# Simple-Robotics/LoIK

Hardware: AMD Instinct MI355X
Metric: IK solves/sec to 1e-6 residual, Talos humanoid, batch=65536 per GPU (higher is better)
Workload: dtype f64

## Files before the change

loik_amd/csrc/loik_flat.hpp:

```cpp
#pragma once

#include "loik_lean.hpp"

namespace loikb {

constexpr int FLAT_RED = 8;
constexpr int FLAT_PART = 8;
constexpr int FLAT_JMP = 5;
constexpr int FLAT_MAXA = 16;
constexpr int FOLDW = 10;
constexpr int FLAT_COUNTERS_SLOT_HITS = 12;
constexpr int FLAT_NA_SMALL = 10;
constexpr int FSLOT_ROWS = 8;

struct FlatLane {
  int depth;
  int size;
  int jmp[FLAT_JMP];
  int anc[FLAT_MAXA];
  int red[FLAT_RED];
  int helper;
  int part[FLAT_PART];
};

enum : int { FC_LANE = 0, FC_B = 1, FC_Y = 7, FC_ATY = 13, FC_ATYW = 19, FC_ATBW = 25, FC_DY = 31, FC_DLT = 37, FC_ATYF = 43, FC_AW = 49, FC_A = 85,
              FC_VC = FC_DLT , FCD = 121 };
enum : int { FI_BNORM = 0, FI_TGIN, FI_STY, FI_TOLP, FI_TOLD, FI_DYQP, FI_ATDY, FI_UBP, FI_LBM, FI_C1, FI_C2, FI_PRIMAL, FI_DUAL, FI_DX,
             FI_DZ, FI_MULAST, FI_RED , FISC = FI_RED + 16 };

template <int NA>
__host__ __device__ constexpr int flat_xregion()
{
  int n = XROWS * 9;
  if (NA * WAVE + 2 > n) n = NA * WAVE + 2;
  if (WAVE * FOLDW > n) n = WAVE * FOLDW;
  return (n + 1) & ~1;
}
template <int NA> __host__ __device__ constexpr int flat_off_wl() { return flat_xregion<NA>(); }
template <int NA> __host__ __device__ constexpr int flat_off_nbuf() { return flat_off_wl<NA>() + 2 * (NA + 1) * WAVE; }
template <int NA> __host__ __device__ constexpr int flat_off_pbuf() { return flat_off_nbuf<NA>() + WAVE + 2; }
template <int NA> __host__ __device__ constexpr int flat_off_rbuf() { return flat_off_pbuf<NA>() + WAVE + 2; }
template <int NA> __host__ __device__ constexpr int flat_off_tail() { return flat_off_rbuf<NA>() + WAVE; }

template <typename T, int NA>
__host__ __device__ __forceinline__ size_t flat_lds_bytes(int nc, int G, bool a_shared, bool has_hv)
{
  (void)a_shared;
  const size_t per_inst = (size_t)nc * FCD + FISC;
  const size_t n = (size_t)flat_off_tail<NA>() + (has_hv ? (size_t)WAVE * 6 : 0) + (size_t)(WAVE / G) * per_inst;
  return (n * sizeof(T) + 15) & ~(size_t)15;
}

__device__ __forceinline__ size_t fslotA_at(int idx, int ndec, int dsl, int fblk, int G, int k, int jlane)
{
  (void)G;
  return ((size_t)idx * ndec + dsl) * fblk + (size_t)jlane * 8 + k;
}
__device__ __forceinline__ size_t fslotW_at(int idx, int ndec, int dsl, int fblk, int col)
{
  return ((size_t)idx * ndec + dsl) * fblk + col;
}

template <typename T>
__device__ __forceinline__ void se3_compose_left(const T* Ra, const T* ta, T* R, T* t)
{
  T Rn[9], tn[3];
#pragma unroll
  for (int i = 0; i < 3; ++i) {
#pragma unroll
    for (int j = 0; j < 3; ++j) Rn[3 * i + j] = Ra[3 * i] * R[j] + Ra[3 * i + 1] * R[3 + j] + Ra[3 * i + 2] * R[6 + j];
    tn[i] = ta[i] + Ra[3 * i] * t[0] + Ra[3 * i + 1] * t[1] + Ra[3 * i + 2] * t[2];
  }
#pragma unroll
  for (int k = 0; k < 9; ++k) R[k] = Rn[k];
#pragma unroll
  for (int k = 0; k < 3; ++k) t[k] = tn[k];
}

template <typename T>
__device__ __forceinline__ void flat_world_placement(T* xb, int lane, int jlane, const unsigned int* jrow4, int njmp, T* R, T* t)
{
#pragma unroll 1
  for (int r = 0; r < njmp; ++r) {
    {
      const int jr = (int)(((r < 4 ? jrow4[0] : jrow4[1]) >> (8 * (r & 3))) & 0xFFu);
      T Ra[9], ta[3];
      tail_sync();
      if (jlane < 9) xb[WAVE * 9 + jlane] = (jlane == 0 || jlane == 4 || jlane == 8) ? T(1) : T(0);
#pragma unroll
      for (int k = 0; k < 9; ++k) xb[lane * 9 + k] = R[k];
      tail_sync();
#pragma unroll
      for (int k = 0; k < 9; ++k) Ra[k] = xb[jr * 9 + k];
      tail_sync();
      if (jlane < 3) xb[WAVE * 9 + jlane] = T(0);
#pragma unroll
      for (int k = 0; k < 3; ++k) xb[lane * 9 + k] = t[k];
      tail_sync();
#pragma unroll
      for (int k = 0; k < 3; ++k) ta[k] = xb[jr * 9 + k];
      se3_compose_left(Ra, ta, R, t);
    }
  }
  tail_sync();
}

template <typename T>
__device__ __forceinline__ void flat_subtree_sum(T* rows, int lane, int jlane, int lim, int size, int nscan, const T* x, T* S)
{
  tail_sync();
  if (jlane < 6) rows[WAVE * 6 + jlane] = T(0);
  T B[6];
#pragma unroll
  for (int k = 0; k < 6; ++k) { B[k] = x[k]; S[k] = T(0); }
  int pos = lane;
  for (int k = 0; k < nscan; ++k) {
    tail_sync();
#pragma unroll
    for (int c = 0; c < 6; ++c) rows[lane * 6 + c] = B[c];
    tail_sync();
    const bool take = (size >> k) & 1;
    const int ra = take ? pos : WAVE;
    const int nx = lane + (1 << k);
    const int rb = nx < lim ? nx : WAVE;
    T a[6], b[6];
#pragma unroll
    for (int c = 0; c < 6; ++c) a[c] = rows[ra * 6 + c];
#pragma unroll
    for (int c = 0; c < 6; ++c) b[c] = rows[rb * 6 + c];
#pragma unroll
    for (int c = 0; c < 6; ++c) { S[c] += a[c]; B[c] += b[c]; }
    pos += take ? (1 << k) : 0;
  }
}

template <typename T>
__device__ __forceinline__ void flat_path_sum(T* rows, int lane, int jlane, const unsigned int* jrow4, int njmp, T* y)
{
  tail_sync();
  if (jlane < 6) rows[WAVE * 6 + jlane] = T(0);
#pragma unroll 1
  for (int r = 0; r < njmp; ++r) {
    {
      const int jr = (int)(((r < 4 ? jrow4[0] : jrow4[1]) >> (8 * (r & 3))) & 0xFFu);
      tail_sync();
#pragma unroll
      for (int c = 0; c < 6; ++c) rows[lane * 6 + c] = y[c];
      tail_sync();
      T a[6];
#pragma unroll
      for (int c = 0; c < 6; ++c) a[c] = rows[jr * 6 + c];
#pragma unroll
      for (int c = 0; c < 6; ++c) y[c] += a[c];
    }
  }
}

template <typename T>
__device__ __forceinline__ void actinv_force(const T* R, const T* t, const T* F, T* o)
{
  T c[3], d[3];
  cross3(t, F, c);
#pragma unroll
  for (int k = 0; k < 3; ++k) d[k] = F[3 + k] - c[k];
  mat3t_vec(R, F, o);
  mat3t_vec(R, d, o + 3);
}

template <typename T, int NMAX>
__device__ __forceinline__ void flat_fold8(T* rows, int lane, int gbase, int jlane, int lgG, const T* in, T* out)
{
  tail_sync();
  T* row = rows + lane * FOLDW;
#pragma unroll
  for (int q = 0; q < 8; ++q) row[q] = in[q];
  tail_sync();
  const int q = jlane & 7;
  const bool ismax = q < NMAX;
  const int nparts = 1 << (lgG - 3);
  {
    const T* col = rows + (gbase + (jlane >> 3)) * FOLDW + q;
    T a[8];
#pragma unroll
    for (int u = 0; u < 8; ++u) a[u] = col[u * nparts * FOLDW];
    const T m = tmax(tmax(tmax(a[0], a[1]), tmax(a[2], a[3])), tmax(tmax(a[4], a[5]), tmax(a[6], a[7])));
    T sm = a[0];
#pragma unroll
    for (int u = 1; u < 8; ++u) sm += a[u];
    row[8] = (NMAX >= 8 || ismax) ? m : sm;
  }
  tail_sync();
  {
    const T* col = rows + (gbase + q) * FOLDW + 8;
    T a[8];
#pragma unroll
    for (int p = 0; p < 8; ++p) a[p] = (p < 4 || lgG > 5) ? col[p * 8 * FOLDW] : T(0);
    const T m = tmax(tmax(tmax(a[0], a[1]), tmax(a[2], a[3])), tmax(tmax(a[4], a[5]), tmax(a[6], a[7])));
    T sm = a[0];
#pragma unroll
    for (int p = 1; p < 8; ++p) sm += a[p];
    row[9] = (NMAX >= 8 || ismax) ? m : sm;
  }
  tail_sync();
#pragma unroll
  for (int u = 0; u < 8; ++u) out[u] = rows[(gbase + u) * FOLDW + 9];
}

__device__ __forceinline__ unsigned int opaque(unsigned int x) { asm volatile("" : "+v"(x)); return x; }
__device__ __forceinline__ int unpack8(const unsigned int* w, int k) { return (int)((opaque(w[k >> 2]) >> (8 * (k & 3))) & 0xFFu); }
__device__ __forceinline__ int unpack16(const unsigned int* w, int k) { return (int)((opaque(w[k >> 1]) >> (16 * (k & 1))) & 0xFFFFu); }
// ... 537 lines not shown
        put_rows();
        tail_sync();
        scan_step(kk);
      }
      if (kk >= nscan) {
        tail_sync();
        part_v();
      } else {
        put_rows();
        tail_sync();
        const int wv = 1 << kk;
        const bool take0 = (size >> kk) & 1, take1 = (size >> (kk + 1)) & 1;
        const int p1 = pos + (take0 ? wv : 0);
        const int r0 = take0 ? pos : WAVE, r1 = take1 ? p1 : WAVE, r2 = take1 ? p1 + wv : WAVE;
        T a[6], b[6], c2[6];
#pragma unroll
        for (int c = 0; c < 6; ++c) a[c] = xb[r0 * 6 + c];
#pragma unroll
        for (int c = 0; c < 6; ++c) b[c] = xb[r1 * 6 + c];
#pragma unroll
        for (int c = 0; c < 6; ++c) c2[c] = xb[r2 * 6 + c];
        part_v();
#pragma unroll
        for (int c = 0; c < 6; ++c) SEn[c] += a[c] + (b[c] + c2[c]);
      }
      tail_sync();
      TAIL_TP(4)
#pragma unroll
      for (int k = 0; k < 6; ++k) Fw[k] = (P.rho + href_s) * SEn[k] - P.rho * SE[k];
      if (has_hv) {
#pragma unroll
        for (int k = 0; k < 6; ++k) Fw[k] -= shv[lane * 6 + k];
      }
      for (int c = 0; c < L.nc; ++c) {
        const T* c_ = cdi + c * cs;
        const T m = cmask(c);
#pragma unroll
        for (int k = 0; k < 6; ++k) Fw[k] += m * c_[FC_ATYF + k];
      }
      actinv_force(R0, t0, Fw, fi);
      si = dot6_halves(Sw, Fw);
#pragma unroll
      for (int k = 0; k < 6; ++k) SE[k] = SEn[k];
    }
    TAIL_TP(5)
    {
      T df[6];
#pragma unroll
      for (int k = 0; k < 6; ++k) df[k] = fi[k] - f[k];
      l_dfis = mass * inf6(df);
      si += w;
      l_stf = tabs(si);
      l_dstf = tabs(si - s);
      s = si;
#pragma unroll
      for (int k = 0; k < 6; ++k) f[k] = fi[k];
    }
    TAIL_TP(3)
    T red[8];
    {
      T in[8] = {tmax(l_prt, l_prs), tmax(l_dualv, l_stf), tmax(l_dvis, l_dnu), l_dz,
                 tmax(l_dfis, tmax(l_dyis, l_dw)), tmax(l_dg, l_dstf), l_up, l_lm};
      flat_fold8<T, 6>(xb, lane, gbase, jlane, lgG, in, red);
    }
    T ntol_p = T(0), ntol_d = T(0);
    if (P.tol_rel != T(0)) {
      T in2[8] = {tmax(l_av, l_nu), tmax(tmax(l_hrefv, l_g), l_stf), T(0), T(0), T(0), T(0), T(0), T(0)}, r2[8];
      flat_fold8<T, 8>(xb, lane, gbase, jlane, lgG, in2, r2);
      ntol_p = r2[0]; ntol_d = r2[1];
    }
    TAIL_TP(6)
    const T primal = red[0], dual = red[1], dx = red[2], dz = red[3], dyqp = red[4], atdy = red[5], ubp = red[6], lbm = red[7];
    const T mu_used = mu;
    const bool fixed = P.mode & MODE_FIXED_ITERS;
    const bool in_tail = (status & ST_TAIL) != 0;
    const bool logic = act && !fixed && !in_tail;
    const T tol_p = P.tol_abs + P.tol_rel * tmax(ntol_p, isc[FI_BNORM]);
    const T tol_d = P.tol_abs + P.tol_rel * tmax(ntol_d, P.Hv_inf_norm);
    const int itn = iter + (act ? 1 : 0);
    const bool conv = logic && (primal < tol_p) && (dual < tol_d);
    const bool feas_chk = logic && itn > 1;
    const bool c1 = atdy <= P.tol_primal_inf * dyqp, c2 = (ubp + lbm) <= P.tol_primal_inf * dyqp;
    const bool infeas = feas_chk && c1 && c2;
    const bool enter_tail = infeas && !conv;
    const bool upd = logic && !conv && !infeas;
    const bool mu_up = upd && (primal > T(10) * dual), mu_dn = upd && !mu_up && (dual > T(10) * primal);
    const bool tail_stop = !(dx >= P.tol_tail_solve || dz >= P.tol_tail_solve) || itn >= P.max_iter;
    const bool stop = act && (conv || ((enter_tail || in_tail) && tail_stop) || ((upd || fixed) && itn + 1 >= P.max_iter));
    iter = itn;
    status |= (conv ? ST_CONVERGED : 0) | (infeas ? ST_PRIMAL_INF : 0) | (enter_tail ? ST_TAIL : 0) | (stop ? ST_DONE : 0);
    tail_it = enter_tail ? 0 : (act && in_tail ? tail_it + 1 : tail_it);
    mu = mu_up ? mu * T(10) : (mu_dn ? mu * T(0.1) : mu);
    kexp += (mu_up ? 1 : 0) - (mu_dn ? 1 : 0);
    nflip += (mu_up || mu_dn) ? 1 : 0;
    done = done || stop;
    const bool finishing = stop;
    const bool leaving = done && has_inst;
    if (LOG) {
      T inl[8] = {l_prt, l_prs, l_stf, l_dualv, T(0), T(0), T(0), T(0)}, rl[8];
      flat_fold8<T, 8>(xb, lane, gbase, jlane, lgG, inl, rl);
      const int row = itn - 1;
      if (act && !in_tail && jlane == 0 && row < Bf.log_cap) {
        const double vals[9] = {(double)rl[0], (double)rl[1], (double)primal, (double)rl[2], (double)rl[3], (double)dual,
                                (double)mu_used, (double)(P.mu_scale * mu_used), (double)mu_used};
#pragma unroll
        for (int l = 0; l < 9; ++l) Bf.log[((size_t)l * Bf.log_B + lidx) * Bf.log_cap + row] = vals[l];
      }
    }
    if (__any(finishing || enter_tail)) {
      if ((finishing || enter_tail) && jlane == 0) {
        isc[FI_PRIMAL] = primal; isc[FI_DUAL] = dual; isc[FI_DX] = dx; isc[FI_DZ] = dz; isc[FI_MULAST] = mu_used;
        if (logic) { isc[FI_TOLP] = tol_p; isc[FI_TOLD] = tol_d; }
        if (feas_chk) {
          isc[FI_C1] = (T)(c1 ? 1 : 0); isc[FI_C2] = (T)(c2 ? 1 : 0); isc[FI_DYQP] = dyqp; isc[FI_ATDY] = atdy; isc[FI_UBP] = ubp; isc[FI_LBM] = lbm;
        }
      }
    }
    if (__any(finishing)) {
      T in1[8] = {l_prt, l_prs, l_stf, l_dvis, l_dnu, l_dfis, l_dyis, l_dw}, in2[8] = {l_av, l_nu, l_hrefv, l_g, l_dualv, T(0), T(0), T(0)};
      T r1[8], r2[8];
      flat_fold8<T, 8>(xb, lane, gbase, jlane, lgG, in1, r1);
      flat_fold8<T, 8>(xb, lane, gbase, jlane, lgG, in2, r2);
      if (finishing && jlane == 0) {
#pragma unroll
        for (int k = 0; k < 8; ++k) isc[FI_RED + k] = r1[k];
#pragma unroll
        for (int k = 0; k < 5; ++k) isc[FI_RED + 8 + k] = r2[k];
      }
      tail_sync();
    }
    if (leaving) {
      store_instance();
      need_load = true;
    }
    TAIL_TP(7)
  }
#ifdef LOIKB_TAIL_PROF
  if (blockIdx.x == 0 && threadIdx.x == 0) {
    for (int k = 0; k < 8; ++k) g_tail_prof[k] = prof_[k];
    for (int k = 8; k < 12; ++k) g_tail_prof[2 + k] = prof_[k];
    g_tail_prof[8] = n_wave_iters;
    g_tail_prof[9] = (clock64() - clk0_) * 100000ull / (wall_clock64() - wall0_ + 1);
  }
#endif
  if (lane == 0) atomicAdd(&Bf.counters[5], n_wave_iters);
  if (jlane == 0) {
    atomicAdd(&Bf.counters[6], n_slot_loads >> 16);
    atomicAdd(&Bf.counters[FLAT_COUNTERS_SLOT_HITS], n_slot_hits);
    atomicOr(&Bf.counters[LEAN_DECADES_SEEN], n_slot_loads & 0xFFFFu);
  }
}

template <typename T, int NA>
__global__ void __launch_bounds__(WAVE)
k_fslots(const Params<T> P, const Bufs<T> Bf, const JointDesc* __restrict__ jd, const TailTopo* __restrict__ topo,
         const int* __restrict__ child_list, const FlatLane* __restrict__ fl, int maxdepth, int nanc, int frows, int njmp,
         const int* __restrict__ slots, int nslots, int G, T* __restrict__ fslots, int kexp_lo, int ndec, int dw0, int nw,
         unsigned int* __restrict__ fmask)
{
  extern __shared__ __attribute__((aligned(16))) unsigned char smem_raw[];
  const Layout& L = P.L;
  constexpr int HX = 22;
  T* xch = reinterpret_cast<T*>(smem_raw);
  T* swt = xch + (WAVE + 1) * HX;
  T* ata_l = swt + (WAVE + 1) * 6;
  T* mutab = ata_l + (size_t)(WAVE / G) * P.L.nc * 21;
  T* lb = xch;
  const int lane = threadIdx.x;
  const int ipw = WAVE / G;
  const int sub = lane / G, jlane = lane % G, gbase = sub * G;
  const int nblk = gridDim.x, xcd = blockIdx.x & 7, rnd = blockIdx.x >> 3;
  const int blk = xcd * (nblk >> 3) + (xcd < (nblk & 7) ? xcd : (nblk & 7)) + rnd;
  const int idx = blk * ipw + sub;
  const bool has_inst = idx < nslots;
  const bool isj_lane = jlane < L.nb;
  const bool isj = has_inst && isj_lane;
  const int jl = isj_lane ? jlane : 0;
  const int sidx = slots[has_inst ? idx : 0];
  char* ip = lane_ptr<T>(Bf.tiles, L, sidx);
  int depth, fcol, arow[NA];
  T Sw[6];
  bool has_parent;
  int cslot;
  T base0[21];
  {
    const JointDesc d = jd[jl + 1];
    const FlatLane F = fl[jlane];
    depth = isj_lane ? F.depth : 0;
    fcol = F.helper >> 8;
    has_parent = !(d.flags & JF_PARENT_ROOT);
    cslot = isj_lane ? d.cslot : -1;
    unsigned int jrow4[(FLAT_JMP + 3) / 4] = {0u, 0u};
#pragma unroll
    for (int r = 0; r < FLAT_JMP; ++r) jrow4[r >> 2] |= (unsigned int)(F.jmp[r] >= 0 ? gbase + F.jmp[r] : WAVE) << (8 * (r & 3));
#pragma unroll
    for (int k = 0; k < NA; ++k) arow[k] = (k < FLAT_MAXA && F.anc[k] >= 0) ? gbase + F.anc[k] : WAVE;
    const char* rec = ip + (size_t)jl * JREC * pair_bytes<T>();
    const typename Vec2<T>::type cs = ldp<T>(rec, JP_CS);
    T R0[9], t0[3];
    joint_xform<T>(d, rec, cs.x, cs.y, R0, t0);
    if (!isj_lane) {
#pragma unroll
      for (int k = 0; k < 9; ++k) R0[k] = (k % 4 == 0) ? T(1) : T(0);
#pragma unroll
      for (int k = 0; k < 3; ++k) t0[k] = T(0);
    }
    flat_world_placement<T>(xch, lane, jlane, jrow4, njmp, R0, t0);
    const bool rev = d.flags & JF_REVOLUTE;
    const int jflags_h = d.flags;
    const T pitch_h = (d.flags & JF_HELICAL) ? (T)d.pitch : T(0);
    T ax[3], ra3[3], c[3];
#pragma unroll
    for (int k = 0; k < 3; ++k) ax[k] = isj_lane ? (T)d.axis[k] : T(0);
    mat3_vec(R0, ax, ra3);
    cross3(t0, ra3, c);
#pragma unroll
    for (int k = 0; k < 3; ++k) { Sw[k] = rev ? c[k] : ra3[k]; Sw[3 + k] = rev ? ra3[k] : T(0); }
    if (jflags_h & JF_HELICAL) {
#pragma unroll
      for (int k = 0; k < 3; ++k) Sw[k] += pitch_h * ra3[k];
    }
#pragma unroll
    for (int k = 0; k < 6; ++k) swt[lane * 6 + k] = Sw[k];
    if (lane < 6) swt[WAVE * 6 + lane] = T(0);
    {
      const T mass = (!isj_lane || (d.flags & JF_MASSLESS)) ? T(0) : T(1);
      T hb[21];
#pragma unroll
      for (int a = 0; a < 6; ++a)
#pragma unroll
        for (int b2 = a; b2 < 6; ++b2)
          hb[sym(a, b2)] = mass * ((a == b2 ? P.rho : T(0)) + (P.href_tab ? P.href_tab[(size_t)(jl + 1) * HREF_ROW + 6 * a + b2] : P.Href[6 * a + b2]));
      congr_sym(R0, t0, hb, base0);
    }
    if (cslot >= 0) {
      const char* crec = ip + (size_t)(L.off_c + cslot * L.crec) * pair_bytes<T>();
      T at[21], atw[21];
      for (int k = 0; k < 21; ++k)
        at[k] = (P.mode & MODE_A_SHARED) ? Bf.uni[L.nc * 36 + cslot * 21 + k]
                                         : *reinterpret_cast<const T*>(crec + (size_t)(CP_ATA + k / 2) * pair_bytes<T>() + (k & 1) * sizeof(T));
      congr_sym(R0, t0, at, atw);
#pragma unroll
      for (int k = 0; k < 21; ++k) ata_l[(sub * L.nc + cslot) * 21 + k] = atw[k];
    }
  }
  const TailTopo tp = topo[jl + 1];
  constexpr int NCH_REG = 3;
  int chl[NCH_REG];
#pragma unroll
  for (int c = 0; c < NCH_REG; ++c) chl[c] = (isj_lane && c < tp.nchild) ? gbase + child_list[tp.child_start + c] : WAVE;
  if (lane < ndec && lane < 16) mutab[lane] = (T)flat_decade_mu((double)P.mu0, kexp_lo + lane);
  tail_sync();
  if (lane < HX) xch[WAVE * HX + lane] = T(0);
  if (fmask != nullptr && has_inst && jlane == 0) fmask[sidx] = (nw >= 32 ? 0xFFFFu : ((1u << nw) - 1u)) << dw0;
  {
    const int lag = maxdepth - depth;
    tail_sync();
    for (int st = 0; st < maxdepth + nw - 1; ++st) {
      const int dsl = dw0 + st - lag;
      const bool on = isj && depth > 0 && dsl >= dw0 && dsl < dw0 + nw;
      T hh[21];
#pragma unroll
      for (int k = 0; k < 21; ++k) hh[k] = base0[k];
      const bool any2 = __any(on && tp.nchild > 1), any3 = __any(on && tp.nchild > 2);
      if (on) {
#pragma unroll
        for (int c = 0; c < NCH_REG; ++c) {
          if ((c == 1 && !any2) || (c == 2 && !any3)) continue;
          const T* x = xch + chl[c] * HX;
#pragma unroll
          for (int k = 0; k < 21; ++k) hh[k] += x[k];
        }
#pragma unroll 1
        for (int c = NCH_REG; c < tp.nchild; ++c) {
          const T* x = xch + (gbase + child_list[tp.child_start + c]) * HX;
#pragma unroll
          for (int k = 0; k < 21; ++k) hh[k] += x[k];
        }
      }
      tail_sync();
      if (on) {
        const T mu = mutab[dsl];
        const T mu_eq = P.mu_scale * mu, mu_in = mu;
        if (cslot >= 0) {
          const T* at = ata_l + (sub * L.nc + cslot) * 21;
#pragma unroll
          for (int k = 0; k < 21; ++k) hh[k] += mu_eq * at[k];
        }
        T U[6], UD[6];
        symv(hh, Sw, U);
        const T dinv = T(1) / (dot6_halves(Sw, U) + mu_in);
#pragma unroll
        for (int k = 0; k < 6; ++k) UD[k] = U[k] * dinv;
#pragma unroll
        for (int k = 0; k < 6; ++k) fslots[fslotA_at(sidx, ndec, dsl, frows, G, k, jlane)] = UD[k];
        fslots[fslotA_at(sidx, ndec, dsl, frows, G, 6, jlane)] = dinv;
        if (has_parent) {
          T* x = xch + lane * HX;
#pragma unroll
          for (int a = 0; a < 6; ++a)
#pragma unroll
            for (int b2 = a; b2 < 6; ++b2) x[sym(a, b2)] = hh[sym(a, b2)] - UD[a] * U[b2];
        }
      }
      tail_sync();
    }
  }
  lb[NA * WAVE + lane] = T(0);
  __builtin_amdgcn_s_waitcnt(0);
  tail_sync();
  for (int dsl = dw0; dsl < dw0 + nw; ++dsl) {
    T UDw[6], dinv = T(0);
#pragma unroll
    for (int k = 0; k < 6; ++k) UDw[k] = isj ? fslots[fslotA_at(sidx, ndec, dsl, frows, G, k, jlane)] : T(0);
    if (isj) dinv = fslots[fslotA_at(sidx, ndec, dsl, frows, G, 6, jlane)];
    T Lc[NA], Wc[NA];
#pragma unroll
    for (int k = 0; k < NA; ++k) {
      Lc[k] = dot6_halves(swt + arow[k] * 6, UDw);
      Wc[k] = T(0);
    }
    tail_sync();
#pragma unroll
    for (int k = 0; k < NA; ++k) lb[k * WAVE + lane] = Lc[k];
    tail_sync();
#pragma unroll
    for (int k = NA - 1; k >= 0; --k) {
      T acc = Lc[k];
#pragma unroll
      for (int k2 = k + 1; k2 < NA; ++k2) acc += lb[k * WAVE + arow[k2]] * Wc[k2];
      Wc[k] = (k < depth - 1) ? -acc : T(0);
    }
    tail_sync();
    if (isj) {
      const size_t base = fslotW_at(sidx, ndec, dsl, frows, fcol);
#pragma unroll
      for (int k = 0; k < NA; ++k)
        if (k < depth - 1) fslots[base + k] = Wc[k];
      fslots[base + depth - 1] = dinv;
    }
  }
}

template <typename T>
__global__ void k_rebuild_ud(char* tiles, Layout L, const JointDesc* __restrict__ jd, const T* __restrict__ uni, T rho, T mu_scale,
                             const T* __restrict__ href_tab, int a_shared, int B, T* __restrict__ scratch)
{
  const int b = blockIdx.x * blockDim.x + threadIdx.x;
  if (b >= B) return;
  char* lp = lane_ptr<T>(tiles, L, b);
  char* srec = lp + (size_t)L.off_s * pair_bytes<T>();
  if (*elem_ptr<T>(srec, SP_TAG, 0) != T(-2)) return;
  const T mu = *elem_ptr<T>(srec, SP_ST, 1);
  const T mu_eq = mu_scale * mu, mu_in = mu;
  T* o = scratch + (size_t)b * L.nb * 21;
  for (int i = 1; i <= L.nb; ++i) {
    for (int r = 0; r < 6; ++r)
      for (int c = r; c < 6; ++c)
        o[(i - 1) * 21 + sym(r, c)] = (jd[i].flags & JF_MASSLESS) ? T(0) : ((r == c ? rho : T(0)) + href_tab[(size_t)i * HREF_ROW + 6 * r + c]);
    if (jd[i].cslot >= 0) {
      const int cs = jd[i].cslot;
      for (int k = 0; k < 21; ++k) {
        const T a = a_shared ? uni[L.nc * 36 + cs * 21 + k]
                             : *elem_ptr<T>(lp + (size_t)(L.off_c + cs * L.crec) * pair_bytes<T>(), CP_ATA + k / 2, k & 1);
        o[(i - 1) * 21 + k] += mu_eq * a;
      }
    }
  }
  for (int i = L.nb; i >= 1; --i) {
    const JointDesc d = jd[i];
    T hh[21], U[6], UD[6], R[9], t[3], part[21];
    for (int k = 0; k < 21; ++k) hh[k] = o[(i - 1) * 21 + k];
    const int a0 = (d.flags & JF_REVOLUTE) ? 3 : 0;
    const T ax0 = (T)d.axis[0], ax1 = (T)d.axis[1], ax2 = (T)d.axis[2];
    for (int k = 0; k < 6; ++k) U[k] = hh[sym(k, a0)] * ax0 + hh[sym(k, a0 + 1)] * ax1 + hh[sym(k, a0 + 2)] * ax2;
    T sus = ax0 * U[a0] + ax1 * U[a0 + 1] + ax2 * U[a0 + 2];
    if (d.flags & JF_HELICAL) {
      const T ph = (T)d.pitch;
      for (int k = 0; k < 6; ++k) U[k] += ph * (hh[sym(k, 0)] * ax0 + hh[sym(k, 1)] * ax1 + hh[sym(k, 2)] * ax2);
      sus = (ax0 * U[3] + ax1 * U[4] + ax2 * U[5]) + ph * (ax0 * U[0] + ax1 * U[1] + ax2 * U[2]);
    }
    const T dd = T(1) / (sus + mu_in);
    for (int k = 0; k < 6; ++k) UD[k] = U[k] * dd;
    char* rec = lp + (size_t)(i - 1) * JREC * pair_bytes<T>();
    st6<T>(rec, JP_UD, UD);
    st_hi<T>(rec, JP_R, dd);
    {
      T vv[6], ff[6], hv[6];
      ld6<T>(rec, JP_V, vv);
      ld6<T>(rec, JP_F, ff);
      symv(hh, vv, hv);
      for (int k = 0; k < 6; ++k) ff[k] -= hv[k];
      st6<T>(rec, JP_P, ff);
    }
    if (d.parent == 0) continue;
    for (int r = 0; r < 6; ++r)
      for (int c = r; c < 6; ++c) hh[sym(r, c)] -= UD[r] * U[c];
    const typename Vec2<T>::type cs = ldp<T>(rec, JP_CS);
    joint_xform<T>(d, rec, cs.x, cs.y, R, t);
    congr_sym(R, t, hh, part);
    for (int k = 0; k < 21; ++k) o[(d.parent - 1) * 21 + k] += part[k];
  }
  *elem_ptr<T>(srec, SP_TAG, 0) = mu;
  *elem_ptr<T>(srec, SP_ST, 0) = (T)((int)*elem_ptr<T>(srec, SP_ST, 0) | ST_PFULL);
}

}
```

loik_amd/csrc/loik_host.hip:

```cpp
#include "loik_device.hpp"
#include "loik_tail.hpp"
#include "loik_lean.hpp"
#include "loik_flat.hpp"
#include "loik_flat2.hpp"
#include "loik_passes.hpp"
#include "loik_pose.hpp"
#include "loik_pose_tasks.hpp"
#include "loik_flat_inst.hpp"
#ifdef LOIKB_FLAT_SEPARATE_TU
LOIKB_FLAT2_INSTANCES(LOIKB_FLAT2_DECL)
LOIKB_FLAT1_INSTANCES(LOIKB_FLAT1_DECL)
#ifdef LOIKB_TAIL_PROF
int loikb_flat_prof_read(unsigned long long* out, int which, int reset);
#endif
#endif

#include "../../include/loik_amd.h"
#include "../../include/loik_amd_pose.h"
#include "../../include/loik_amd_limits.h"
#include "../../include/loik_amd_tasks.h"

#include <algorithm>
#include <chrono>
#include <cmath>
// ... 1736 lines not shown
    int k03 = 99, k97 = 99;
    for (int k = 0; k < 32; ++k) {
      cum += S->end_hist[k];
      if (k03 == 99 && cum * 100 >= 3ull * S->end_hist_n) k03 = k - 16;
      if (k97 == 99 && cum * 100 >= 97ull * S->end_hist_n) k97 = k - 16;
    }
    wlo = std::min(0, k03); whi = std::max(0, k97);
  }
  else if (S->tune.flat_build == 2 && win_ok && n >= 49152) {
    wlo = 0; whi = 4;
  }
  const int lo = std::max(wlo, F.kexp_lo), hi = std::min(whi, F.kexp_lo + F.ndec - 1);
  if (hi >= lo && (hi - lo + 1) < F.ndec) { F.dw0 = lo - F.kexp_lo; F.nw = hi - lo + 1; }
  else if (S->tune.flat_build == 2) F.mur = 0;
}

template <typename T>
static int launch_flat_kernel(TailCtx<T>& X, FlatLaunch& F)
{
  loikb_solver_impl* S = X.S; Chunk* C = X.C;
  const int n = X.n, has_hv = F.has_hv;
  const int cus = (int)(F.cu_sh + 0.5);
  if (one_per_wave(F.kind)) {
    if (C->d_aux == nullptr) HIPCHK(hipMalloc((void**)&C->d_aux, 4 * sizeof(void*)));
    const void* auxh[4] = {S->d_topo, S->d_child_list, C->d_fmask, nullptr};
    if (memcmp(auxh, C->aux_h, sizeof(auxh)) != 0) {
      memcpy(C->aux_h, auxh, sizeof(auxh));
      HIPCHK(hipStreamSynchronize(C->stream));
      HIPCHK(hipMemcpy(C->d_aux, C->aux_h, sizeof(auxh), hipMemcpyHostToDevice));
    }
  }
  const Params<double>& Pd = *reinterpret_cast<const Params<double>*>(&X.P);
  const Bufs<double>& Bd = *reinterpret_cast<const Bufs<double>*>(&X.Bf);
  const FlatVariant v = flat_variant(F.kind, href_mode(S), F.slice > 0, S->opt.logging != 0, F.mur);
  const int quantum = v.sliced ? F.slice : 0;
  if (F.kind == FlatKind::Flat2) {
    const size_t lds2 = flat2_lds_bytes<FLAT_NA_SMALL>(S->nc, has_hv != 0, F.mur == 1);
    int per_cu = (int)std::min<size_t>((size_t)8, (160 * 1024) / lds2);
    if (S->tune.lean_wg_per_cu > 0) per_cu = std::min(per_cu, S->tune.lean_wg_per_cu);
    F.grid = dim3((unsigned)std::min(n, per_cu * cus));
    const int win_bits = (int)(((F.nw >= 16 ? 0xFFFFu : ((1u << F.nw) - 1u)) << F.dw0) & 0xFFFFu);
    hipLaunchKernelGGL(flat_kernel(FLAT2_TABLE, v, FLAT_NA_SMALL), F.grid, dim3(WAVE), lds2, C->stream, Pd, Bd, (const JointDesc*)S->d_jd, (const FlatLane*)S->flat.d_lanes,
                       F.nanc, S->flat.nscan, S->flat.njmp, C->d_ring, n, (const double*)C->d_fslots, F.frows, F.kexp_lo, F.ndec, (double)S->Href[0],
                       (int)((unsigned int)has_hv | ((unsigned int)(S->maxdepth & 0xFF) << 8) | ((unsigned int)win_bits << 16)), C->ring_cap - 1,
                       quantum, (double*)C->d_park, flat2_park_stride(S->nc, true), (const void* const*)C->d_aux);
  } else if (F.kind == FlatKind::Flat1) {
    auto lds_of = [&](int bufs) { return F.small_na ? flat1_lds_bytes<FLAT_NA_SMALL>(S->nc, has_hv != 0, bufs) : flat1_lds_bytes<FLAT_MAXA>(S->nc, has_hv != 0, bufs); };
    const int one_buf = F.mur != 1 && std::min<size_t>(8, (160 * 1024) / lds_of(1)) > std::min<size_t>(8, (160 * 1024) / lds_of(2));
    const size_t lds1 = lds_of(one_buf ? 1 : 2);
    int per_cu1 = (int)std::min<size_t>(8, (160 * 1024) / lds1);
    if (S->tune.lean_wg_per_cu > 0) per_cu1 = std::min(per_cu1, S->tune.lean_wg_per_cu);
    F.grid = dim3((unsigned)std::min(n, per_cu1 * cus));
    hipLaunchKernelGGL(flat_kernel(FLAT1_TABLE, v, F.small_na ? FLAT_NA_SMALL : FLAT_MAXA), F.grid, dim3(WAVE), lds1, C->stream, Pd, Bd, (const JointDesc*)S->d_jd,
                       (const FlatLane*)S->flat.d_lanes, F.nanc, S->flat.nscan, S->flat.njmp, C->d_ring, n, (const double*)C->d_fslots, F.frows,
                       F.kexp_lo, F.ndec, (double)S->Href[0], has_hv | (one_buf ? 2 : 0) | ((S->maxdepth & 0xFF) << 8), C->ring_cap - 1, quantum,
                       (const void* const*)C->d_aux);
  } else {
    const size_t flds = F.small_na ? flat_lds_bytes<T, FLAT_NA_SMALL>(S->nc, X.G, S->a_shared, has_hv) : flat_lds_bytes<T, FLAT_MAXA>(S->nc, X.G, S->a_shared, has_hv);
    int lgG = 3;
    while ((1 << lgG) < X.G) ++lgG;
    F.grid = dim3((unsigned)std::min((n + X.ipw - 1) / X.ipw, (int)std::min<size_t>(4, (160 * 1024) / flds) * cus));
    auto* kernel = S->opt.logging ? (F.small_na ? k_flat<T, FLAT_NA_SMALL, true> : k_flat<T, FLAT_MAXA, true>)
                                  : (F.small_na ? k_flat<T, FLAT_NA_SMALL> : k_flat<T, FLAT_MAXA>);
    hipLaunchKernelGGL(kernel, F.grid, dim3(WAVE), flds, C->stream, X.P, X.Bf, (const JointDesc*)S->d_jd, (const FlatLane*)S->flat.d_lanes, F.nanc,
                       S->flat.nscan, S->flat.njmp, (const int*)C->d_ring, n, lgG, (const T*)C->d_fslots, F.frows, F.kexp_lo, F.ndec, (T)S->Href[0], has_hv);
  }
  HIPCHK(hipGetLastError());
  return LOIKB_OK;
}

template <typename T>
static int flat_read_back(TailCtx<T>& X, const FlatLaunch& F, OrderUse use, bool order_pass, bool small_finish, bool queue_ready, int* next)
{
  loikb_solver_impl* S = X.S; Chunk* C = X.C;
  const int n_first = X.n, n_cur = X.n_cur;
  const hipEvent_t ev_first = queue_ready ? S->ev_t0 : C->ev_k0;
  float ms = 0.f, t0 = 0.f, hms = 0.f;
  HIPCHK(hipEventElapsedTime(&ms, ev_first, C->ev_k1));
  if (!queue_ready) HIPCHK(hipEventElapsedTime(&t0, S->ev_t0, C->ev_k0));
  if (!X.small_flat) HIPCHK(hipEventElapsedTime(&hms, ev_first, C->ev_k2));
  X.iters += C->h_counters[1];
  if (C->h_counters[FLAT_COUNTERS_ERR]) {
    g_last_error = (C->h_counters[FLAT_COUNTERS_ERR] & 4u) ? "internal: the flat engine's dynamic LDS does not start at LDS address 0 (lds_abs)"
                                                           : "internal: a wavefront of the flat engine gave up waiting on its work queue";
    return LOIKB_ERR_STATE;
  }
  C->stats.lean_requeues += (int)C->h_counters[LEAN_Q_REQUEUES];
  const unsigned int escaped = C->h_counters[2];
  C->stats.flat_built += (int)C->h_counters[FLAT_COUNTERS_BUILT];
  {
    std::lock_guard<std::mutex> lock(S->alloc_mu);
    record_decades(S, C->h_counters[LEAN_DECADES_SEEN], F.kexp_lo, escaped);
    if (order_pass) {
      if (S->end_hist_epoch != S->solve_serial) { S->end_hist_epoch = S->solve_serial; S->end_hist_n = 0; for (int k = 0; k < 32; ++k) S->end_hist[k] = 0; }
      for (int k = 0; k < 32; ++k) { S->end_hist[k] += C->h_counters[ORDER_DEC_HIST + k]; S->end_hist_n += C->h_counters[ORDER_DEC_HIST + k]; }
    }
    if (F.mur == 2) {
      for (int k = 0; k < 32; ++k)
        if (C->h_counters[FLAT_COUNTERS_DEC + k]) { S->seen_lo = std::min(S->seen_lo, k - 16); S->seen_hi = std::max(S->seen_hi, k - 16); }
    }
    S->ud_stale = true;
  }
  C->stats.hslots_ms += hms;
  if (C->h_counters[FLAT_COUNTERS_DRY])
    C->stats.queue_dry_ms += (double)(unsigned int)(C->h_counters[FLAT_COUNTERS_TDRY] - C->h_counters[FLAT_COUNTERS_T0]) * 1e-5;
  if (one_per_wave(F.kind) && X.whole_set && n_first == n_cur) judge_order(S, C, n_cur, use, (double)ms - (double)hms);
  if (S->tune.trace)
    fprintf(stderr, "[loikb] flat engine: %6d instances on %u workgroups, done at %8.3f ms (slots %6.3f ms)  "
                    "inst-iters %9u  wave-iters %7u  slot loads %7u (+ %u served from LDS)  escaped %u  still iterating %u\n",
            n_first, F.grid.x, ms, hms, C->h_counters[1], C->h_counters[5], C->h_counters[6],
            C->h_counters[FLAT_COUNTERS_SLOT_HITS], escaped, C->h_counters[3]);
  C->stats.lean_escaped += (int)escaped;
  C->tail_iv.emplace_back(t0, t0 + ms);
  X.total_ms = ms; X.n = (int)C->h_counters[3]; X.list = next;
  if (X.n == 0 && X.whole_set && X.cur == 0 && n_first == n_cur && S->chunks.size() == 1) { C->stats.n_unfinished = (int)C->h_counters[4]; C->unfinished_counted = true; C->small_finished = small_finish; }
  return LOIKB_OK;
}

template <typename T>
static int launch_flat(TailCtx<T>& X)
{
  loikb_solver_impl* S = X.S; Chunk* C = X.C;
  Params<T>& P = X.P;
  const int n = X.n, n_cur = X.n_cur;
  const bool small_flat = X.small_flat, whole_set = X.whole_set;
  FlatLaunch F;
  F.kind = flat_kind(S); F.nanc = S->flat.nanc; F.small_na = F.nanc <= FLAT_NA_SMALL; F.has_hv = S->Hv_inf_norm != 0.0;
  F.frows = S->flat.fblk;
  F.cu_sh = std::max(1.0, S->ncu * ((double)C->B / (double)S->B));
  F.ndec = X.ndec; F.kexp_lo = X.kexp_lo; F.dw0 = 0;
  const bool can_build2 = S->tune.flat_build && F.kind == FlatKind::Flat2 && C->d_fmask != nullptr && !S->opt.logging && !S->per_link && href_is_scalar(S);
  F.mur = flat_any_mu(S) ? 1 : (can_build2 ? 2 : 0);
  if (F.mur == 1) { F.ndec = 1; F.kexp_lo = 0; }
  if (F.mur == 2) { F.ndec = S->plan.ndec; F.kexp_lo = S->plan.kexp_lo; }
  const size_t need = (size_t)n_cur * F.ndec * F.frows * sizeof(T);
  if (need > C->fslots_bytes) { g_last_error = "internal: decade-slot buffer of the flat engine smaller than the chunk"; return LOIKB_ERR_STATE; }
  P.max_launch_iters = S->opt.max_iter + 1;
  const int mode_keep = P.mode;
  if (whole_set && S->zero_state && S->tune.flat_zero_state) P.mode |= MODE_ZERO_STATE;
  const bool queue_ready = small_flat && C->queue_ready && n_cur == S->B;
  C->queue_ready = false;
  if (!queue_ready && small_flat) hipLaunchKernelGGL(k_queue_init_iota, grid1(std::max(C->ring_cap, NCOUNTERS)), dim3(256), 0, C->stream, C->d_ring, C->ring_cap, C->d_slots, n_cur, C->d_counters, NCOUNTERS);
  else if (!queue_ready) HIPCHK(hipMemsetAsync(C->d_counters, 0, NCOUNTERS * sizeof(unsigned int), C->stream));
  if (!queue_ready) HIPCHK(hipEventRecord(C->ev_k0, C->stream));
  OrderUse use;
  int rc = take_up_order(S, C, !small_flat && whole_set && X.list == C->d_slots && n == n_cur && one_per_wave(F.kind), true, n_cur, &use);
  if (rc) return rc;
  F.slice = flat_launch_slice(S, C, F.kind, F.mur, n, n_cur, use.ordered);
  F.nw = F.ndec;
  if (F.mur == 2) flat_table_window(S, F, n);
  if (F.mur == 0) { F.ndec = X.ndec; F.kexp_lo = X.kexp_lo; F.nw = F.ndec; F.dw0 = 0; }
  if (F.ndec > 0) {
    const dim3 hgrid((unsigned)((n + X.ipw - 1) / X.ipw));
    const size_t slds = (std::max((size_t)(WAVE + 1) * 22, (size_t)((F.small_na ? FLAT_NA_SMALL : FLAT_MAXA) + 1) * WAVE) + (size_t)(WAVE + 1) * 6 +
                         (size_t)X.ipw * S->nc * 21 + 16) * sizeof(T);
    auto* fslots = F.small_na ? k_fslots<T, FLAT_NA_SMALL> : k_fslots<T, FLAT_MAXA>;
    hipLaunchKernelGGL(fslots, hgrid, dim3(WAVE), slds, C->stream, P, X.Bf, (const JointDesc*)S->d_jd, (const TailTopo*)S->d_topo,
                       (const int*)S->d_child_list, (const FlatLane*)S->flat.d_lanes, S->maxdepth, F.nanc, F.frows, S->flat.njmp, X.list, n,
                       X.G, (T*)C->d_fslots, F.kexp_lo, F.ndec, F.dw0, F.nw, F.mur == 2 ? C->d_fmask : (unsigned int*)nullptr);
    HIPCHK(hipGetLastError());
  }
  if (!small_flat) HIPCHK(hipEventRecord(C->ev_k2, C->stream));
  if (!small_flat) hipLaunchKernelGGL(k_ring_fill, grid1(C->ring_cap), dim3(256), 0, C->stream, C->d_ring, C->ring_cap, X.list, n, C->d_counters);
  if ((rc = launch_flat_kernel(X, F))) return rc;
  P.mode = mode_keep;
  int* next = (X.list == C->d_slots) ? C->d_slots2 : C->d_slots;
  const bool small_finish = small_flat && S->tune.small_finish;
  if (small_finish)
    hipLaunchKernelGGL(k_small_finish<T>, dim3(1), dim3(256), 0, C->stream, X.A.tiles, S->L, X.list, n, next, C->d_counters, NCOUNTERS, C->h_counters);
  else
    hipLaunchKernelGGL(k_list_unfinished<T>, grid1(n), dim3(256), 0, C->stream, X.A.tiles, S->L, X.list, n, next, C->d_counters + 3);
  HIPCHK(hipGetLastError());
  C->stats.launches++; C->stats.tail_launches++; C->stats.lean_launches++; C->stats.flat_launches++;
  if (F.kind == FlatKind::Flat2) C->stats.flat_split_launches++;
  HIPCHK(hipEventRecord(C->ev_k1, C->stream));
  const bool order_pass = !small_flat && S->tune.flat_order && whole_set && n == n_cur && one_per_wave(F.kind) && !(S->opt.flags & LOIKB_OPT_FIXED_ITERS);
  if (!order_pass && !small_finish) HIPCHK(hipMemcpyAsync(C->h_counters, C->d_counters, NCOUNTERS * sizeof(unsigned int), hipMemcpyDeviceToHost, C->stream));
  if (order_pass && (rc = leave_order<T>(S, C, X.A, n_cur, true))) return rc;
  HIPCHK(hipStreamSynchronize(C->stream));
  return flat_read_back(X, F, use, order_pass, small_finish, queue_ready, next);
}

template <typename T>
static int launch_lean(TailCtx<T>& X)
{
  loikb_solver_impl* S = X.S; Chunk* C = X.C;
  Params<T>& P = X.P;
  const Bufs<T>& Bf = X.Bf;
  const int n = X.n, n_cur = X.n_cur, G = X.G, ipw = X.ipw, ndec = X.ndec, kexp_lo = X.kexp_lo;
  const int* list = X.list;
  const bool whole_set = X.whole_set, per_link = S->per_link;
  const size_t need = (size_t)n_cur * ndec * HSLOT_PAIRS * G * 2 * sizeof(T);
  if (need > C->hslots_bytes) { g_last_error = "internal: decade-slot buffer smaller than the chunk"; return LOIKB_ERR_STATE; }
  const int waves_cu = S->plan.lean_waves_cu;
  const int ltw = S->plan.lean_wg_waves;
  const size_t lds = ltw * lean_lds_bytes<T>(S->nc, G, S->a_shared);
  if (lds > 64 * 1024) {
    HIPCHK(hipFuncSetAttribute((const void*)k_lean<T, true>, hipFuncAttributeMaxDynamicSharedMemorySize, (int)lds));
    HIPCHK(hipFuncSetAttribute((const void*)k_lean<T, false>, hipFuncAttributeMaxDynamicSharedMemorySize, (int)lds));
    HIPCHK(hipFuncSetAttribute((const void*)k_lean<T, false, true>, hipFuncAttributeMaxDynamicSharedMemorySize, (int)lds));
  }
  const int wg_per_cu = S->tune.lean_wg_per_cu > 0 ? S->tune.lean_wg_per_cu : waves_cu / ltw;
  const int wg_cap = wg_per_cu * std::max(1, (int)(S->ncu * ((double)C->B / (double)S->B) + 0.5));
  HIPCHK(hipEventRecord(C->ev_k0, C->stream));
  OrderUse use;
  int rc = take_up_order(S, C, whole_set && list == C->d_slots && n == n_cur, whole_set, n_cur, &use);
  if (rc) return rc;
  P.max_launch_iters = S->opt.max_iter + 1;
  const int wg_needed = (n + ipw * ltw - 1) / (ipw * ltw);
  const dim3 grid((unsigned)std::min(wg_needed, wg_cap));
  HIPCHK(hipMemsetAsync(C->d_counters, 0, NCOUNTERS * sizeof(unsigned int), C->stream));
  const dim3 hgrid((unsigned)((n + ipw - 1) / ipw));
  const size_t hlds = (size_t)(WAVE + 1) * 22 * sizeof(T);
  auto* hslots = per_link ? k_hslots<T, false, true> : S->href_diag ? k_hslots<T, true> : k_hslots<T, false>;
  hipLaunchKernelGGL(hslots, hgrid, dim3(WAVE), hlds, C->stream, P, Bf, (const JointDesc*)S->d_jd, (const TailTopo*)S->d_topo,
                     (const int*)S->d_child_list, S->maxdepth, S->maxchild, list, n, G, (T*)C->d_hslots, kexp_lo, ndec);
  HIPCHK(hipEventRecord(C->ev_k2, C->stream));
  hipLaunchKernelGGL(k_ring_fill, grid1(C->ring_cap), dim3(256), 0, C->stream, C->d_ring, C->ring_cap, list, n, C->d_counters);
  auto* lean = per_link ? k_lean<T, false, true> : S->href_diag ? k_lean<T, true> : k_lean<T, false>;
  hipLaunchKernelGGL(lean, grid, dim3(WAVE * ltw), lds, C->stream, P, Bf, (const JointDesc*)S->d_jd, (const TailTopo*)S->d_topo,
                     (const int*)S->d_child_list, S->maxdepth, S->maxchild, C->d_ring, n, G, (const T*)C->d_hslots, kexp_lo, ndec, S->multi_from);
  HIPCHK(hipGetLastError());
  int* next = (list == C->d_slots) ? C->d_slots2 : C->d_slots;
  hipLaunchKernelGGL(k_list_unfinished<T>, grid1(n), dim3(256), 0, C->stream, X.A.tiles, S->L, list, n, next, C->d_counters + 3);
  HIPCHK(hipGetLastError());
  HIPCHK(hipEventRecord(C->ev_k1, C->stream));
  HIPCHK(hipMemcpyAsync(C->h_counters, C->d_counters, NCOUNTERS * sizeof(unsigned int), hipMemcpyDeviceToHost, C->stream));
  const bool lean_orders = S->tune.flat_order && whole_set && n == n_cur && !(S->opt.flags & LOIKB_OPT_FIXED_ITERS);
  if (lean_orders && (rc = leave_order<T>(S, C, X.A, n_cur, false))) return rc;
  HIPCHK(hipStreamSynchronize(C->stream));
  float ms = 0.f, t0 = 0.f, hms = 0.f;
  HIPCHK(hipEventElapsedTime(&ms, C->ev_k0, C->ev_k1));
  if (lean_orders) judge_order(S, C, n_cur, use, (double)ms);
  HIPCHK(hipEventElapsedTime(&t0, S->ev_t0, C->ev_k0));
  X.iters += C->h_counters[1];
  const unsigned int escaped = C->h_counters[2];
  {
    std::lock_guard<std::mutex> lock(S->alloc_mu);
    record_decades(S, C->h_counters[LEAN_DECADES_SEEN], kexp_lo, escaped);
  }
  C->stats.lean_requeues += (int)C->h_counters[LEAN_Q_REQUEUES];
  HIPCHK(hipEventElapsedTime(&hms, C->ev_k0, C->ev_k2));
  C->stats.hslots_ms += hms;
  if (S->tune.trace)
    fprintf(stderr, "[loikb] lean engine: %6d instances on %u workgroups, done at %8.3f ms"
                    "  inst-iters %9u  wave-iters %7u slot loads %7u  escaped %u  still iterating %u  requeued %u\n",
            n, grid.x, ms, C->h_counters[1], C->h_counters[5], C->h_counters[6], escaped,
            C->h_counters[3], C->h_counters[LEAN_Q_REQUEUES]);
  C->stats.launches++; C->stats.tail_launches++; C->stats.lean_launches++;
  X.total_ms = ms; X.n = (int)C->h_counters[3]; X.list = next;
  C->tail_iv.emplace_back(t0, t0 + ms);
  C->stats.lean_escaped += (int)escaped;
  return LOIKB_OK;
}

template <typename T>
static int launch_tail_kernel(TailCtx<T>& X, int tw, size_t lds)
{
  loikb_solver_impl* S = X.S; Chunk* C = X.C;
  const int n = X.n, n_cur = X.n_cur;
  const int cu_share = std::max(1, (int)(S->ncu * (TAIL_WAVES / tw) * ((double)C->B / (double)S->B) + 0.5));
  X.P.max_launch_iters = S->opt.max_iter + 1;
  const int wg_needed = (n + X.ipw * tw - 1) / (X.ipw * tw);
  const dim3 grid((unsigned)std::min(wg_needed, cu_share));
  HIPCHK(hipMemsetAsync(C->d_counters, 0, NCOUNTERS * sizeof(unsigned int), C->stream));
  HIPCHK(hipEventRecord(C->ev_k0, C->stream));
  const bool tail_whole = X.whole_set && X.list == C->d_slots && n == n_cur && !(S->opt.flags & LOIKB_OPT_FIXED_ITERS) && S->tune.flat_order;
  OrderUse use;
  int rc = take_up_order(S, C, tail_whole, tail_whole, n_cur, &use);
  if (rc) return rc;
  auto* kernel = S->href_diag ? k_tail<T, true> : k_tail<T, false>;
  hipLaunchKernelGGL(kernel, grid, dim3(WAVE * tw), lds, C->stream, X.P, X.Bf, (const JointDesc*)S->d_jd, (const TailTopo*)S->d_topo,
                     (const int*)S->d_child_list, S->maxdepth, S->maxchild, X.list, n, X.G);
  HIPCHK(hipGetLastError());
  HIPCHK(hipEventRecord(C->ev_k1, C->stream));
  HIPCHK(hipMemcpyAsync(C->h_counters, C->d_counters, NCOUNTERS * sizeof(unsigned int), hipMemcpyDeviceToHost, C->stream));
  if (tail_whole && (rc = leave_order<T>(S, C, X.A, n_cur, false))) return rc;
  HIPCHK(hipStreamSynchronize(C->stream));
  float ms = 0.f, t0 = 0.f;
  HIPCHK(hipEventElapsedTime(&ms, C->ev_k0, C->ev_k1));
  HIPCHK(hipEventElapsedTime(&t0, S->ev_t0, C->ev_k0));
  if (tail_whole) judge_order(S, C, n_cur, use, (double)ms);
  C->tail_iv.emplace_back(t0, t0 + ms);
  X.total_ms += ms;
  X.iters += C->h_counters[1];
  if (S->tune.trace)
    fprintf(stderr, "[loikb] tail launch: %6d instances on %u workgroups  %8.3f ms  inst-iters %9u (%.1f M/s)"
                    "  wave-iters %7u H-rebuild %3.0f%%\n",
            n, grid.x, ms, C->h_counters[1], C->h_counters[1] / ms / 1e3,
            C->h_counters[5], 100.0 * C->h_counters[6] / (C->h_counters[5] ? C->h_counters[5] : 1));
  C->stats.launches++; C->stats.tail_launches++;
  return LOIKB_OK;
}

template <typename T>
int run_tail(loikb_solver_impl* S, Chunk* C, Params<T>& P, int cur, int n_cur, int n_live, double* ms_out,
             unsigned long long* iters_out, bool whole_set = false)
{
  loikb_solver_impl::Set& A = C->set[cur];
  const int nw = (n_cur + WAVE - 1) / WAVE;
  const bool flat_here = flat_applicable(S) && (P.mode & MODE_CACHE_H);
  const bool flat_1pw = one_per_wave(flat_kind(S));
  const bool small_flat = whole_set && cur == 0 && S->chunks.size() == 1 && flat_1pw && flat_here && n_cur <= S->tune.flat_small_batch &&
                          n_cur >= std::max(1, S->tune.flat_min_batch);
  if (whole_set && !small_flat) {
    hipLaunchKernelGGL(k_list_iota, grid1(n_cur), dim3(256), 0, C->stream, C->d_slots, n_cur);
  } else if (!whole_set) {
// ... 1936 lines not shown
```

Measured before the change: 7.065 million.

## Keep decade-slot factors in registers and double-buffer the fslots back-substitution rounds

The fslots kernel now processes decades in groups of four. The per-decade UD/dinv factors stay in registers instead of being written to global memory and read back, so the scratch region fslotA is removed. Back-substitution rounds alternate between two LDS buffers, which drops some barriers, and a waves-per-EU occupancy hint is added. The cost is more registers for the group arrays, a larger LDS region, and the tree sweep running once per group rather than once overall.

```diff
diff --git a/loik_amd/csrc/loik_flat.hpp b/loik_amd/csrc/loik_flat.hpp
--- a/loik_amd/csrc/loik_flat.hpp
+++ b/loik_amd/csrc/loik_flat.hpp
@@ -12,6 +12,7 @@
 constexpr int FLAT_COUNTERS_SLOT_HITS = 12;
 constexpr int FLAT_NA_SMALL = 10;
 constexpr int FSLOT_ROWS = 8;
+constexpr int FSLOT_GRP = 4;
 
 struct FlatLane {
   int depth;
@@ -51,11 +52,6 @@
   return (n * sizeof(T) + 15) & ~(size_t)15;
 }
 
-__device__ __forceinline__ size_t fslotA_at(int idx, int ndec, int dsl, int fblk, int G, int k, int jlane)
-{
-  (void)G;
-  return ((size_t)idx * ndec + dsl) * fblk + (size_t)jlane * 8 + k;
-}
 __device__ __forceinline__ size_t fslotW_at(int idx, int ndec, int dsl, int fblk, int col)
 {
   return ((size_t)idx * ndec + dsl) * fblk + col;
@@ -899,7 +895,46 @@
 }
 
 template <typename T, int NA>
-__global__ void __launch_bounds__(WAVE)
+__host__ __device__ constexpr int fslots_waves()
+{
+  return sizeof(T) == 8 ? (NA <= FLAT_NA_SMALL ? 2 : 1) : (NA <= FLAT_NA_SMALL ? 3 : 2);
+}
+
+template <typename T, int NA>
+__device__ __forceinline__ void fslots_round(const T* swt, T* lb, const int* arow, int depth, int lane, bool isj, const T* r, T* __restrict__ o)
+{
+  T Lc[NA], Wc[NA];
+#pragma unroll
+  for (int k = 0; k < NA; ++k) {
+    Lc[k] = dot6_halves(swt + arow[k] * 6, r);
+    Wc[k] = T(0);
+  }
+#pragma unroll
+  for (int k = 0; k < NA; ++k) lb[k * WAVE + lane] = Lc[k];
+  tail_sync();
+#pragma unroll
+  for (int k = NA - 1; k >= 0; --k) {
+    T acc = Lc[k];
+#pragma unroll
+    for (int k2 = k + 1; k2 < NA; ++k2) acc += lb[k * WAVE + arow[k2]] * Wc[k2];
+    Wc[k] = (k < depth - 1) ? -acc : T(0);
+  }
+  if (isj) {
+#pragma unroll
+    for (int k = 0; k < NA; ++k)
+      if (k < depth - 1) o[k] = Wc[k];
+    o[depth - 1] = r[6];
+  }
+}
+
+template <int NA>
+__host__ __device__ constexpr int fslots_xregion()
+{
+  return (WAVE + 1) * 22 > 2 * (NA + 1) * WAVE ? (WAVE + 1) * 22 : 2 * (NA + 1) * WAVE;
+}
+
+template <typename T, int NA>
+__global__ void __launch_bounds__(WAVE) __attribute__((amdgpu_waves_per_eu(fslots_waves<T, NA>())))
 k_fslots(const Params<T> P, const Bufs<T> Bf, const JointDesc* __restrict__ jd, const TailTopo* __restrict__ topo,
          const int* __restrict__ child_list, const FlatLane* __restrict__ fl, int maxdepth, int nanc, int frows, int njmp,
          const int* __restrict__ slots, int nslots, int G, T* __restrict__ fslots, int kexp_lo, int ndec, int dw0, int nw,
@@ -907,9 +942,9 @@
 {
   extern __shared__ __attribute__((aligned(16))) unsigned char smem_raw[];
   const Layout& L = P.L;
-  constexpr int HX = 22;
+  constexpr int HX = 22, LBS = (NA + 1) * WAVE;
   T* xch = reinterpret_cast<T*>(smem_raw);
-  T* swt = xch + (WAVE + 1) * HX;
+  T* swt = xch + fslots_xregion<NA>();
   T* ata_l = swt + (WAVE + 1) * 6;
   T* mutab = ata_l + (size_t)(WAVE / G) * P.L.nc * 21;
   T* lb = xch;
@@ -998,14 +1033,23 @@
   for (int c = 0; c < NCH_REG; ++c) chl[c] = (isj_lane && c < tp.nchild) ? gbase + child_list[tp.child_start + c] : WAVE;
   if (lane < ndec && lane < 16) mutab[lane] = (T)flat_decade_mu((double)P.mu0, kexp_lo + lane);
   tail_sync();
-  if (lane < HX) xch[WAVE * HX + lane] = T(0);
   if (fmask != nullptr && has_inst && jlane == 0) fmask[sidx] = (nw >= 32 ? 0xFFFFu : ((1u << nw) - 1u)) << dw0;
-  {
-    const int lag = maxdepth - depth;
+  const int lag = maxdepth - depth;
+#pragma unroll 1
+  for (int g0 = 0; g0 < nw; g0 += FSLOT_GRP) {
+    const int gn = nw - g0 < FSLOT_GRP ? nw - g0 : FSLOT_GRP;
+    T rw[FSLOT_GRP][7];
+#pragma unroll
+    for (int g = 0; g < FSLOT_GRP; ++g)
+#pragma unroll
+      for (int k = 0; k < 7; ++k) rw[g][k] = T(0);
     tail_sync();
-    for (int st = 0; st < maxdepth + nw - 1; ++st) {
-      const int dsl = dw0 + st - lag;
-      const bool on = isj && depth > 0 && dsl >= dw0 && dsl < dw0 + nw;
+    if (lane < HX) xch[WAVE * HX + lane] = T(0);
+    tail_sync();
+    for (int st = 0; st < maxdepth + gn - 1; ++st) {
+      const int dg = st - lag;
+      const int dsl = dw0 + g0 + dg;
+      const bool on = isj && depth > 0 && dg >= 0 && dg < gn;
       T hh[21];
 #pragma unroll
       for (int k = 0; k < 21; ++k) hh[k] = base0[k];
@@ -1040,8 +1084,13 @@
 #pragma unroll
         for (int k = 0; k < 6; ++k) UD[k] = U[k] * dinv;
 #pragma unroll
-        for (int k = 0; k < 6; ++k) fslots[fslotA_at(sidx, ndec, dsl, frows, G, k, jlane)] = UD[k];
-        fslots[fslotA_at(sidx, ndec, dsl, frows, G, 6, jlane)] = dinv;
+        for (int g = 0; g < FSLOT_GRP; ++g) {
+          if (dg == g) {
+#pragma unroll
+            for (int k = 0; k < 6; ++k) rw[g][k] = UD[k];
+            rw[g][6] = dinv;
+          }
+        }
         if (has_parent) {
           T* x = xch + lane * HX;
 #pragma unroll
@@ -1052,39 +1101,12 @@
       }
       tail_sync();
     }
-  }
-  lb[NA * WAVE + lane] = T(0);
-  __builtin_amdgcn_s_waitcnt(0);
-  tail_sync();
-  for (int dsl = dw0; dsl < dw0 + nw; ++dsl) {
-    T UDw[6], dinv = T(0);
-#pragma unroll
-    for (int k = 0; k < 6; ++k) UDw[k] = isj ? fslots[fslotA_at(sidx, ndec, dsl, frows, G, k, jlane)] : T(0);
-    if (isj) dinv = fslots[fslotA_at(sidx, ndec, dsl, frows, G, 6, jlane)];
-    T Lc[NA], Wc[NA];
-#pragma unroll
-    for (int k = 0; k < NA; ++k) {
-      Lc[k] = dot6_halves(swt + arow[k] * 6, UDw);
-      Wc[k] = T(0);
-    }
-    tail_sync();
-#pragma unroll
-    for (int k = 0; k < NA; ++k) lb[k * WAVE + lane] = Lc[k];
-    tail_sync();
-#pragma unroll
-    for (int k = NA - 1; k >= 0; --k) {
-      T acc = Lc[k];
-#pragma unroll
-      for (int k2 = k + 1; k2 < NA; ++k2) acc += lb[k * WAVE + arow[k2]] * Wc[k2];
-      Wc[k] = (k < depth - 1) ? -acc : T(0);
-    }
-    tail_sync();
-    if (isj) {
-      const size_t base = fslotW_at(sidx, ndec, dsl, frows, fcol);
-#pragma unroll
-      for (int k = 0; k < NA; ++k)
-        if (k < depth - 1) fslots[base + k] = Wc[k];
-      fslots[base + depth - 1] = dinv;
+    lb[NA * WAVE + lane] = T(0);
+    lb[LBS + NA * WAVE + lane] = T(0);
+#pragma unroll
+    for (int g = 0; g < FSLOT_GRP; ++g) {
+      if (g < gn)
+        fslots_round<T, NA>(swt, lb + (g & 1) * LBS, arow, depth, lane, isj, rw[g], fslots + fslotW_at(sidx, ndec, dw0 + g0 + g, frows, fcol));
     }
   }
 }
diff --git a/loik_amd/csrc/loik_host.hip b/loik_amd/csrc/loik_host.hip
--- a/loik_amd/csrc/loik_host.hip
+++ b/loik_amd/csrc/loik_host.hip
@@ -1912,7 +1912,7 @@
   if (F.mur == 0) { F.ndec = X.ndec; F.kexp_lo = X.kexp_lo; F.nw = F.ndec; F.dw0 = 0; }
   if (F.ndec > 0) {
     const dim3 hgrid((unsigned)((n + X.ipw - 1) / X.ipw));
-    const size_t slds = (std::max((size_t)(WAVE + 1) * 22, (size_t)((F.small_na ? FLAT_NA_SMALL : FLAT_MAXA) + 1) * WAVE) + (size_t)(WAVE + 1) * 6 +
+    const size_t slds = ((size_t)(F.small_na ? fslots_xregion<FLAT_NA_SMALL>() : fslots_xregion<FLAT_MAXA>()) + (size_t)(WAVE + 1) * 6 +
                          (size_t)X.ipw * S->nc * 21 + 16) * sizeof(T);
     auto* fslots = F.small_na ? k_fslots<T, FLAT_NA_SMALL> : k_fslots<T, FLAT_MAXA>;
     hipLaunchKernelGGL(fslots, hgrid, dim3(WAVE), slds, C->stream, P, X.Bf, (const JointDesc*)S->d_jd, (const TailTopo*)S->d_topo,
```

Result: no change. 7.162 million (median of 6 runs) (+1.4%).
